# georgesterpu/avsr-tf1

Hardware: AMD Instinct MI355X
Metric: utterances/sec (train step) at B=64 T_a=500 T_v=75 (higher is better)
Workload: dtype f32; 1 GPU; c4: AV dual-attention (bimodal) video 1x256 + audio 3x256 uni-LSTM, scaled_luong, B=64 T_a=500x80 T_v=75 L=40; utterances_per_gpu=64, global_batch=64, T_a=500, F_a=80, T_v=75, F_v=128, T_dec=40, parallelism=dp1, video_frontend=resnet_cnn, launch=hipgraph, dropout=True

## Files before the change

avsr-tf1_amd/_lib.py:

```python
import ctypes as C
import os

import torch

from . import build as _build

MAX_LAYERS = 4
MAX_MECH = 4
MAX_STACKS = 4

_fp = C.POINTER(C.c_float)
_ip = C.POINTER(C.c_int32)


class AvsrError(RuntimeError):
    pass


class Mat(C.Structure):
    _fields_ = [("ptr", C.c_void_p), ("ld", C.c_int64), ("T", C.c_int32), ("pad_", C.c_int32), ("ldo", C.c_int64)]


class GemmDesc(C.Structure):
    _fields_ = [("A", Mat), ("B", Mat), ("C", Mat), ("bias", C.c_void_p),
# ... 4 lines not shown
                ("alpha_dev", C.c_void_p),
                ("splitk", C.c_int32), ("pad_", C.c_int32),
                ("workspace", C.c_void_p), ("workspace_floats", C.c_int64),
                ("colsum", C.c_void_p), ("colsum_beta", C.c_float), ("pad2_", C.c_int32)]


class RnnLayer(C.Structure):
    _fields_ = [("units", C.c_int32), ("in_dim", C.c_int32), ("hoisted", C.c_int32), ("out_col", C.c_int32),
                ("wt", C.c_void_p), ("w", C.c_void_p), ("bias", C.c_void_p),
                ("gates", C.c_void_p), ("cs", C.c_void_p), ("out", C.c_void_p), ("ld_out", C.c_int64),
                ("state", C.c_void_p), ("h_final", C.c_void_p), ("c_final", C.c_void_p),
                ("dgates", C.c_void_p), ("dstate", C.c_void_p), ("dout", C.c_void_p), ("ld_dout", C.c_int64),
                ("dout_col", C.c_int32), ("residual", C.c_int32), ("hs_seq", C.c_void_p), ("xt_seq", C.c_void_p),
                ("wt2", C.c_void_p), ("w2", C.c_void_p), ("bias2", C.c_void_p), ("rh_seq", C.c_void_p), ("dgates2", C.c_void_p)]


class RnnStack(C.Structure):
    _fields_ = [("B", C.c_int32), ("T", C.c_int32), ("reverse", C.c_int32), ("n_layers", C.c_int32),
                ("cell", C.c_int32), ("pad_", C.c_int32),
                ("len", C.c_void_p), ("dh_final", C.c_void_p), ("dc_final", C.c_void_p),
                ("seed", C.c_void_p), ("keep_in", C.c_float), ("keep_state", C.c_float), ("keep_out", C.c_float),
                ("consumer_keep", C.c_float), ("cell_id_base", C.c_int32), ("consumer_stream", C.c_int32),
                ("consumer_width", C.c_int32), ("pad2_", C.c_int32),
                ("layer", RnnLayer * MAX_LAYERS)]


class RnnLaunch(C.Structure):
    _fields_ = [(n, C.c_int32) for n in ("form", "stacks", "rows_per_group", "rows_per_slice", "launches", "wg_per_xcd", "crossing_edges",
                                         "top_tiles")]


class AttnMech(C.Structure):
    _fields_ = [("type", C.c_int32), ("T", C.c_int32), ("D", C.c_int32), ("chunk", C.c_int32),
                ("len", C.c_void_p), ("keys", C.c_void_p), ("values", C.c_void_p),
                ("values_sb", C.c_int64), ("values_st", C.c_int64),
                ("g", C.c_void_p), ("v", C.c_void_p), ("bq", C.c_void_p),
                ("wq_t", C.c_void_p), ("wq", C.c_void_p), ("watt_t", C.c_void_p), ("watt", C.c_void_p),
                ("scores", C.c_void_p), ("ctx", C.c_void_p), ("pq", C.c_void_p), ("pstat", C.c_void_p),
                ("pctx", C.c_void_p), ("dscores", C.c_void_p), ("dctx", C.c_void_p), ("dpq", C.c_void_p),
                ("pdq", C.c_void_p)]


class DecLayer(C.Structure):
    _fields_ = [("wt", C.c_void_p), ("w", C.c_void_p), ("bias", C.c_void_p), ("gates", C.c_void_p), ("cs", C.c_void_p),
                ("out", C.c_void_p), ("state", C.c_void_p), ("hs_seq", C.c_void_p), ("xin_seq", C.c_void_p),
                ("dgates", C.c_void_p), ("dstate", C.c_void_p), ("cell_id", C.c_int32), ("pad_", C.c_int32),
                ("wt2", C.c_void_p), ("w2", C.c_void_p), ("bias2", C.c_void_p), ("rh_seq", C.c_void_p), ("dgates2", C.c_void_p)]


MAX_DEC_EXTRA = 3


# ... 343 lines not shown
```

avsr-tf1_amd/csrc/persist.h:

```cpp
#pragma once
#include "common.h"
#include "wave.h"
#include "avsr_hip.h"

#define P_HDR 256

namespace avsr {

extern int32_t* g_sync;
extern int64_t g_sync_ints;
extern int g_persist_mode;
extern float* g_persist_scratch;
extern int64_t g_persist_scratch_floats;

struct RnnPlanRec { avsr_rnn_launch* out; int cap, n; };
extern thread_local RnnPlanRec* g_rnn_plan;
static inline void rnn_plan_note(int form, int stacks, int rows_per_group, int rows_per_slice, int B, int wg_per_xcd, int crossing = 0,
                                 int top_tiles = 0) {
  RnnPlanRec* R = g_rnn_plan;
  if (!R) return;
  if (R->n < R->cap)
    R->out[R->n] = avsr_rnn_launch{form, stacks, rows_per_group, rows_per_slice, (B + rows_per_slice - 1) / rows_per_slice, wg_per_xcd, crossing,
                                   top_tiles};
  ++R->n;
}

__device__ __forceinline__ f32x4 ld4_sc1(const float* p) {
  typedef unsigned long long u64;
  const u64 a = __hip_atomic_load(reinterpret_cast<const u64*>(p), __ATOMIC_RELAXED, __HIP_MEMORY_SCOPE_AGENT);
  const u64 b = __hip_atomic_load(reinterpret_cast<const u64*>(p) + 1, __ATOMIC_RELAXED, __HIP_MEMORY_SCOPE_AGENT);
  f32x4 v;
  v[0] = __builtin_bit_cast(float, (unsigned)(a & 0xffffffffu)); v[1] = __builtin_bit_cast(float, (unsigned)(a >> 32));
  v[2] = __builtin_bit_cast(float, (unsigned)(b & 0xffffffffu)); v[3] = __builtin_bit_cast(float, (unsigned)(b >> 32));
  return v;
}
__device__ __forceinline__ void st_sc1(float* p, float v) { __hip_atomic_store(p, v, __ATOMIC_RELAXED, __HIP_MEMORY_SCOPE_AGENT); }

__device__ __forceinline__ bool wait_ge(const int* ctr, int target, int* err) {
  for (int spins = 0; spins < (1 << 21); ++spins) {
    if (__hip_atomic_load(ctr, __ATOMIC_RELAXED, __HIP_MEMORY_SCOPE_AGENT) >= target) return true;
    if ((spins & 1023) == 1023 && __hip_atomic_load(err, __ATOMIC_RELAXED, __HIP_MEMORY_SCOPE_AGENT)) return false;
    __builtin_amdgcn_s_sleep(2);
  }
  __hip_atomic_store(err, 1, __ATOMIC_RELAXED, __HIP_MEMORY_SCOPE_AGENT);
  return false;
}
// ... 46 lines not shown
```

avsr-tf1_amd/csrc/rnn.hip:

```cpp
#include "step.h"
#include "avsr_hip.h"
#include "persist.h"

extern "C" int avsr_step_launch_raw(const void* launch, void* stream);
int avsr_rnn_fwd_persistent(const avsr_rnn_stack* st, int32_t n, void* stream, int dry);
int avsr_rnn_bwd_persistent(const avsr_rnn_stack* st, int32_t n, void* stream, int dry);

static int run_persistent(int (*fn)(const avsr_rnn_stack*, int32_t, void*, int), const avsr_rnn_stack* st, int32_t n, void* stream, int dry = 0) {
  for (int i = 0; i < n; ++i)
    for (int l = 0; l < st[i].n_layers && l < AVSR_MAX_LAYERS; ++l)
      if (st[i].layer[l].residual) return AVSR_ERR_UNSUPPORTED;
  int rc = fn(st, n, stream, dry);
  if (rc != AVSR_ERR_UNSUPPORTED || n == 1) return rc;
  avsr::RnnPlanRec* const rec = avsr::g_rnn_plan;
  const int noted = rec ? rec->n : 0;
  for (int i = 0; i < n; ++i)
    if ((rc = fn(st + i, 1, stream, 1)) != AVSR_OK) { if (rec) rec->n = noted; return rc; }
  if (dry) return AVSR_OK;
  for (int i = 0; i < n; ++i)
    if ((rc = fn(st + i, 1, stream, 0)) != AVSR_OK) return rc;
  return AVSR_OK;
}

static int wavefront_steps(const avsr_rnn_stack* st, int32_t n) {
// ... 290 lines not shown
  }
  return AVSR_OK;
}

extern "C" int avsr_rnn_plan(const avsr_rnn_stack* st, int32_t n, int32_t bwd, int32_t mode, int64_t sync_ints, int64_t scratch_floats,
                             avsr_rnn_launch* out, int32_t cap) {
  using namespace avsr;
  if (!st || n <= 0 || n > AVSR_MAX_STACKS || cap < 0 || (cap > 0 && !out) || sync_ints < 0 || scratch_floats < 0) return AVSR_ERR_ARG;
  for (int i = 0; i < n; ++i)
    if (st[i].n_layers <= 0 || st[i].n_layers > AVSR_MAX_LAYERS || st[i].B <= 0 || st[i].T <= 0) return AVSR_ERR_ARG;
  static int32_t dummy_sync[1];
  static float dummy_scratch[1];
  int32_t* const sync0 = g_sync; const int64_t ints0 = g_sync_ints; const int mode0 = g_persist_mode;
  float* const scr0 = g_persist_scratch; const int64_t floats0 = g_persist_scratch_floats;
  g_sync = sync_ints ? dummy_sync : nullptr; g_sync_ints = sync_ints; g_persist_mode = mode;
  g_persist_scratch = scratch_floats ? dummy_scratch : nullptr; g_persist_scratch_floats = scratch_floats;
  RnnPlanRec R = {out, cap, 0};
  g_rnn_plan = &R;
  const int rc = run_persistent(bwd ? avsr_rnn_bwd_persistent : avsr_rnn_fwd_persistent, st, n, nullptr, 1);
  g_rnn_plan = nullptr;
  g_sync = sync0; g_sync_ints = ints0; g_persist_mode = mode0; g_persist_scratch = scr0; g_persist_scratch_floats = floats0;
  if ((bwd || rc == AVSR_ERR_UNSUPPORTED) && wavefront_tasks(st, n) > STEP_MAX_TASKS) return AVSR_ERR_UNSUPPORTED;
  if (rc == AVSR_ERR_UNSUPPORTED) {
    if (cap > 0) out[0] = avsr_rnn_launch{AVSR_RNN_FORM_PER_STEP, n, 0, 0, wavefront_steps(st, n) * (st[0].cell == 1 ? 2 : 1), 0, 0, 0};
    return 1;
  }
  return rc < 0 ? rc : R.n;
}
```

avsr-tf1_amd/csrc/rnn_persist_bwd.hip:

```cpp
#include "step.h"
#include "avsr_hip.h"
#include "prof.h"
#include "persist.h"

#define B_MAX_TASKS 12
namespace avsr {
float* g_persist_scratch = nullptr;
int64_t g_persist_scratch_floats = 0;
}
extern "C" int avsr_rnn_set_persistent_scratch(float* scratch, int64_t floats) {
  avsr::g_persist_scratch = scratch; avsr::g_persist_scratch_floats = scratch ? floats : 0;
  return AVSR_OK;
}
#define B_CH 8

namespace avsr {

struct BTask {
  const float* w_own; const float* w_up; long ldw_own, ldw_up;
  const int* len;
  const float* gates; const float* cs;
  float* dgates; float* ring; const float* up_dgates;
  float* part;
  float* dx; int kind;
  const float* dout; long dout_sb, dout_st;
  const float* dh_final; const float* dc_final;
  int* prog; const int* prog_up;
  int* ctr; const int* ctr_up;
  int B, T, H, H_up, reverse, nct, nct_up, slot_begin, half, ntile, up_remote;
  const int32_t* seed; float k_st, k_out, k_in; uint32_t r_st, r_out, r_in; int in_W, in_coff;
};
struct BLaunch { int ntask, ngroups, wpx0, wpx1, b0, solo; int* err; int* claim; BTask task[B_MAX_TASKS]; };

__global__ __launch_bounds__(512) void rnn_persist_bwd_kernel(const BLaunch L) {
  __shared__ __attribute__((aligned(16))) float red[8][2][16][16];
  __shared__ int s_slot;
  const int tid = threadIdx.x, lane = tid & 63, wave = tid >> 6;
  const int xcc = __builtin_amdgcn_readfirstlane(xcc_id());
  if (tid == 0) s_slot = __hip_atomic_fetch_add(L.claim + xcc, 1, __ATOMIC_RELAXED, __HIP_MEMORY_SCOPE_AGENT);
  __syncthreads();
  const int slot = __builtin_amdgcn_readfirstlane(s_slot);
  const int g = xcc >> 1, half = xcc & 1;
  if (g >= L.ngroups || slot >= (half ? L.wpx1 : L.wpx0)) return;
  int ti = -1;
#pragma unroll
  for (int i = 0; i < B_MAX_TASKS; ++i)
    if (i < L.ntask && L.task[i].half == half && slot >= L.task[i].slot_begin) ti = i;
// ... 286 lines not shown
  auto publish = [&](int t) {
    asm volatile("s_waitcnt vmcnt(0)" ::: "memory");
    __syncthreads();
    if (tid == 0) {
      __hip_atomic_store(my_prog, T - t, __ATOMIC_RELAXED, __HIP_MEMORY_SCOPE_WORKGROUP);
      if (my_ctr) __hip_atomic_fetch_add(my_ctr + t, 1, __ATOMIC_RELAXED, __HIP_MEMORY_SCOPE_AGENT);
    }
  };

  if (helper) {
    const int K_up = 4 * tk.H_up, ncu = K_up >> 4;
    const int kw = wave & 7, tl = wave >> 3;
    const int b0 = (kw * ncu) / 8, nB = ((kw + 1) * ncu) / 8 - b0;
    f32x4 wB[B_CH];
    {
      const int uu = unit0 + tl * 16 + i;
#pragma unroll
      for (int c = 0; c < B_CH; ++c)
        wB[c] = (c < nB && uu < H) ? ld4(tk.w_up + (long)uu * tk.ldw_up + (b0 + c) * 16 + 4 * q) : f32x4{0.f, 0.f, 0.f, 0.f};
    }
    const __amdgpu_buffer_rsrc_t up_rs = make_rsrc(tk.up_dgates);
    const int up_row = (ab * T * K_up + b0 * 16 + 4 * q) * 4;
    float* const dx_p = tk.dx;
    const float k_in = tk.k_in; const uint32_t r_in = tk.r_in; const int in_W = tk.in_W, in_coff = tk.in_coff;
    for (int t = T - 1; t >= 0; --t) {
      wait_progress(0, t);
      lds_barrier();
      f32x4 aB[B_CH];
      const int o = (aok && t < len_a) ? up_row + (reverse ? len_a - 1 - t : t) * (K_up * 4) : P_OOB;
#pragma unroll
      for (int c = 0; c < B_CH; ++c) aB[c] = ldb_sc1(up_rs, c < nB ? o + c * 64 : P_OOB);
      f32x4 acc0 = {0.f, 0.f, 0.f, 0.f}, acc1 = {0.f, 0.f, 0.f, 0.f};
#pragma unroll
      for (int cc = 0; cc < B_CH; cc += 2)
#pragma unroll
        for (int e = 0; e < 4; ++e) {
          acc0 = __builtin_amdgcn_mfma_f32_16x16x4f32(aB[cc][e], wB[cc][e], acc0, 0, 0, 0);
          acc1 = __builtin_amdgcn_mfma_f32_16x16x4f32(aB[cc + 1][e], wB[cc + 1][e], acc1, 0, 0, 0);
        }
      acc0 += acc1;
#pragma unroll
      for (int r = 0; r < 4; ++r) red[wave][q * 4 + r][i] = acc0[r];
      lds_barrier();
      if (eok && t < len_b) {
        const int tau = reverse ? len_b - 1 - t : t;
        const long bt = (long)b * T + tau;
        float z = 0.f;
#pragma unroll
        for (int w = 0; w < 8; ++w) z += red[(eu >> 4) * 8 + w][er][eu & 15];
        const float v = z * p_drop(drop_on, seedv, r_in, (uint32_t)(bt * in_W + in_coff + u), k_in);
        if (publish_remote) st_sc1(dx_p + bt * H + u, v);
        else dx_p[bt * H + u] = v;
      }
      publish(t);
    }
    return;
  }

  f32x4 wR[TPW][KC];
#pragma unroll
  for (int nt = 0; nt < TPW; ++nt) {
    const int n = (wave * TPW + nt) * 16 + i;
#pragma unroll
    for (int c = 0; c < KC; ++c)
      wR[nt][c] = (n < H && unit0 * 4 + c * 16 + 4 * q < 4 * H) ? ld4(tk.w_own + (long)n * tk.ldw_own + unit0 * 4 + c * 16 + 4 * q)
                                                              : f32x4{0.f, 0.f, 0.f, 0.f};
  }
  float dc_carry = (eok && tk.dc_final) ? tk.dc_final[(long)b * H + u] : 0.f;
  float dh_carry = (eok && tk.dh_final) ? tk.dh_final[(long)b * H + u] : 0.f;
  const __amdgpu_buffer_rsrc_t gates_rs = make_rsrc(tk.gates), cs_rs = make_rsrc(tk.cs), dout_rs = make_rsrc(tk.dout);
  const __amdgpu_buffer_rsrc_t dx_rs = make_rsrc(tk.dx);
  const bool has_dout = tk.dout != nullptr, has_dx = tk.dx != nullptr;
  float* const dgates_p = tk.dgates;
  const __amdgpu_buffer_rsrc_t dgates_rs = make_rsrc(tk.dgates);
  const int dout_b = (int)(b * tk.dout_sb) + u, dout_st = (int)tk.dout_st;
  const float k_st = tk.k_st, k_out = tk.k_out;
  const uint32_t r_st = tk.r_st, r_out = tk.r_out;
// ... 132 lines not shown
  int best = -1, best_cross = 1 << 30, best_load = 1 << 30;
  for (int m = 0; m < (1 << n); ++m) {
    int load[2] = {0, 0}, cross = 0;
    for (int i = 0; i < n; ++i) {
      load[(m >> i) & 1] += cost[i];
      if (upper[i] >= 0 && (((m >> i) ^ (m >> upper[i])) & 1)) cross += ecost ? ecost[i] : 1;
    }
    if (load[0] > cap || load[1] > cap) continue;
    const int mx = load[0] > load[1] ? load[0] : load[1];
    if (cross < best_cross || (cross == best_cross && mx < best_load)) { best = m; best_cross = cross; best_load = mx; }
  }
  if (best < 0) return false;
  for (int i = 0; i < n; ++i) half_out[i] = (best >> i) & 1;
  return true;
}

static_assert(sizeof(BLaunch) <= 4000, "launch descriptor must fit the kernel-argument segment");

}

#include <cstdio>
#include <cstdlib>
#define UNSUP(code) do { if (getenv("AVSR_PERSIST_DEBUG")) fprintf(stderr, "[avsr] persistent BPTT not used: reason %d (rnn_persist_bwd.hip)\n", code); return AVSR_ERR_UNSUPPORTED; } while (0)
static int bwd_persistent(const avsr_rnn_stack* st, int32_t n, void* stream, int dry, bool ksplit);

int avsr_rnn_bwd_persistent(const avsr_rnn_stack* st, int32_t n, void* stream, int dry) {
  if (!(avsr::g_persist_mode & 4)) {
    const int rc = bwd_persistent(st, n, stream, dry, true);
    if (rc != AVSR_ERR_UNSUPPORTED) return rc;
  }
  return bwd_persistent(st, n, stream, dry, false);
}

static int bwd_persistent(const avsr_rnn_stack* st, int32_t n, void* stream, int dry, bool ksplit) {
  const int UWH = 16;
  using namespace avsr;
  int32_t* sync = g_sync; const int64_t sync_ints = g_sync_ints;
  if (!sync || !(g_persist_mode & 2)) return AVSR_ERR_UNSUPPORTED;
  if (ksplit && !g_persist_scratch) return AVSR_ERR_UNSUPPORTED;
  long part_used = 0;
  static thread_local BLaunch L;
  L = BLaunch{};
  double flops = 0.0;
  int cost[B_MAX_TASKS], upper[B_MAX_TASKS], half[B_MAX_TASKS];
  const int B = st[0].B;
  int ngroups = B < 64 ? (B + 15) / 16 : 4;
  for (int i = 0; i < n; ++i) {
    const avsr_rnn_stack& S = st[i];
    if (S.cell != 0 || S.B != B) UNSUP(3);
    const int first = L.ntask;
    for (int l = 0; l < S.n_layers; ++l) {
      const avsr_rnn_layer& Ly = S.layer[l];
      if (L.ntask >= B_MAX_TASKS) UNSUP(4);
      const int H = Ly.units, in = Ly.in_dim;
      const bool top = l + 1 >= S.n_layers;
      if (H % 16 || H > 32 * B_CH || (long)S.B * S.T * H * 4 >= (1L << 29)) UNSUP(5);
      if (!top && (S.layer[l + 1].units % 16 || S.layer[l + 1].units > 32 * B_CH || S.layer[l + 1].in_dim != H)) UNSUP(6);
      if (Ly.dout && (long)S.B * (S.T + 2) * Ly.ld_dout >= (1L << 29)) UNSUP(7);
      const int t_i = L.ntask++;
      BTask& tk = L.task[t_i];
      tk.w_own = Ly.w + (long)in * 4 * H; tk.ldw_own = 4 * H;
      if (!top && !ksplit) { const avsr_rnn_layer& Up = S.layer[l + 1]; tk.w_up = Up.w; tk.ldw_up = 4 * Up.units; tk.H_up = Up.units; tk.up_dgates = Up.dgates; }
      tk.len = S.len; tk.gates = Ly.gates; tk.cs = Ly.cs; tk.dgates = Ly.dgates; tk.ring = Ly.dstate;
      if (Ly.dout) { tk.dout = Ly.dout + Ly.ld_dout + Ly.dout_col; tk.dout_sb = (long)(S.T + 2) * Ly.ld_dout; tk.dout_st = Ly.ld_dout; }
      if (top) { tk.dh_final = S.dh_final; tk.dc_final = S.dc_final; }
      tk.B = S.B; tk.T = S.T; tk.H = H; tk.reverse = S.reverse;
      flops += 2.0 * S.B * S.T * (4.0 * H + (top ? 0.0 : 4.0 * S.layer[l + 1].units)) * H;
// ... 14 lines not shown
        if (!top && !ksplit) { tk.k_in = S.keep_in; tk.r_in = (cid + 1) * 4; tk.in_W = H; tk.in_coff = 0; }
      }
      if (ksplit && !top) {
        if (L.ntask >= B_MAX_TASKS) UNSUP(4);
        const avsr_rnn_layer& Up = S.layer[l + 1];
        const int h_i = L.ntask++;
        BTask& hk = L.task[h_i];
        hk.kind = 1;
        hk.w_up = Up.w; hk.ldw_up = 4 * Up.units; hk.H_up = Up.units; hk.up_dgates = Up.dgates;
        hk.len = S.len; hk.B = S.B; hk.T = S.T; hk.H = H; hk.reverse = S.reverse;
        hk.ntile = 1; hk.nct = H / UWH;
        const long need = (long)S.B * S.T * H;
        if (part_used + need > g_persist_scratch_floats) UNSUP(13);
        hk.dx = g_persist_scratch + part_used; part_used += need;
        tk.dx = hk.dx;
        cost[h_i] = hk.nct; upper[h_i] = h_i + 1;
        if (S.seed) {
          const uint32_t cid = (uint32_t)(S.cell_id_base + l);
          hk.seed = S.seed; hk.k_in = S.keep_in; hk.r_in = (cid + 1) * 4; hk.in_W = H; hk.in_coff = 0;
          hk.k_st = hk.k_out = 1.0f;
        }
      }
    }
    (void)first;
  }
  int ecost[B_MAX_TASKS];
  for (int i = 0; i < L.ntask; ++i) ecost[i] = L.task[i].kind == 1 ? 1 : 3;
  int total_cost = 0;
  for (int i = 0; i < L.ntask; ++i) total_cost += cost[i];
  const int cap = ksplit ? 64 : 28;
  const bool solo = ksplit && B > 64 && total_cost <= cap;
  if (solo) { for (int i = 0; i < L.ntask; ++i) half[i] = 0; ngroups = 8; }
  else if (!assign_halves(cost, upper, L.ntask, cap, half, ksplit ? ecost : nullptr)) UNSUP(9);
  long words = P_HDR + 8;
  int slots[2] = {0, 0};
  for (int pass = 0; pass < 2; ++pass)
    for (int i = 0; i < L.ntask; ++i) {
      BTask& tk = L.task[i];
      if ((tk.kind == 1) != (pass == 1)) continue;
      tk.half = half[i]; tk.slot_begin = slots[half[i]]; slots[half[i]] += tk.nct;
      tk.prog = sync + words; words += 8 * 32;
    }
  for (int i = 0; i < L.ntask; ++i) {
    BTask& tk = L.task[i];
    if (upper[i] < 0) continue;
    BTask& up = L.task[upper[i]];
    tk.prog_up = up.prog; tk.nct_up = up.nct;
    if (up.half != tk.half) {
      tk.up_remote = 1;
      if (!up.ctr) { up.ctr = sync + words; words += (long)ngroups * up.T; }
      tk.ctr_up = up.ctr;
    }
  }
  if (words > sync_ints) UNSUP(10);
  const int slice = solo ? 128 : 64;
  const int wpx = slots[0] > slots[1] ? slots[0] : slots[1];
  if (dry) {
    int crossing = 0, tiles = 1;
    for (int i = 0; i < L.ntask; ++i) { crossing += L.task[i].up_remote; if (L.task[i].ntile > tiles) tiles = L.task[i].ntile; }
    rnn_plan_note(!ksplit ? AVSR_RNN_FORM_BWD_UNIT : solo ? AVSR_RNN_FORM_BWD_KSPLIT_SOLO : AVSR_RNN_FORM_BWD_KSPLIT, n, 16, slice, B, wpx, crossing,
                  ksplit ? 0 : tiles);
    return AVSR_OK;
  }
  L.err = sync; L.claim = sync + P_HDR; L.wpx0 = slots[0]; L.wpx1 = slots[1]; L.solo = solo ? 1 : 0;
  hipStream_t s = (hipStream_t)stream;
  for (int b0 = 0; b0 < B; b0 += slice) {
    const int rows = B - b0 < slice ? B - b0 : slice;
    L.b0 = b0; L.ngroups = (rows + 15) / 16;
    if (avsr::dev_zero(sync + P_HDR, sizeof(int32_t) * (words - P_HDR), s) != hipSuccess) return AVSR_ERR_HIP;
    {
      ProfScope ps(PROF_RNN_PERSIST_BWD, s, flops * rows / B);
      if (ksplit) hipLaunchKernelGGL(rnn_persist_bwdk_kernel, dim3(8 * wpx), dim3(512), 0, s, L);
      else hipLaunchKernelGGL(rnn_persist_bwd_kernel, dim3(8 * wpx), dim3(512), 0, s, L);
    }
    AVSR_CHECK_LAUNCH();
  }
  return AVSR_OK;
}
```

avsr-tf1_amd/model_encoder.py:

```python
import torch
from . import ops
from ._lib import RnnStack
from .config import encoder_cell_id
from .model_base import Batch


class EncoderMixin:
    def _kn(self, prefix):
        return (prefix + "/gates_kernel", prefix + "/gates_bias") if self.gru else (prefix + "/kernel", prefix + "/bias")

    def _keeps(self, s):
        return self.cfg.video_dropout if s == "video" else self.cfg.audio_dropout

    def _sdrop(self, s):
        return self._dropping and min(self._keeps(s)) < 1.0

    def _bdrop(self, blk):
        return self._dropping and min(blk["keep"]) < 1.0

    def _rnn_stack(self, ws, s, d, B, len_t, backward=False):
        cfg = self.cfg
        E = ws["enc"][s]
        st = RnnStack()
        st.B, st.T, st.reverse, st.n_layers, st.cell = B, E["T"], int(d == "bw"), E["nplain"], int(self.gru)
# ... 19 lines not shown
            Ly.w = ops.fptr(self.params, self.P[name].off)
            Ly.bias = ops.fptr(self.params, self.P[bname].off)
            if self.gru:
                cn = f"{s}/enc/{d}/l{cfg.shared_layer(s, l)}/cand_kernel"
                Ly.wt2, Ly.w2 = ops.fptr(self.derived, self.Tr[cn].off), ops.fptr(self.params, self.P[cn].off)
                Ly.bias2 = ops.fptr(self.params, self.P[f"{s}/enc/{d}/l{cfg.shared_layer(s, l)}/cand_bias"].off)
                Ly.rh_seq, Ly.dgates2 = ops.fptr(Ld["rh"]), ops.fptr(Ld["dpc"])
            Ly.gates, Ly.cs = ops.fptr(Ld["gates"]), ops.fptr(Ld["cs"])
            Ly.out, Ly.ld_out = ops.fptr(Ld["out"].t), Ld["out"].D
            Ly.state, Ly.h_final, Ly.c_final = ops.fptr(Ld["state"]), ops.fptr(Ld["hf"]), ops.fptr(Ld["cf"])
            Ly.dgates, Ly.dstate = ops.fptr(Ld["dgates"]), ops.fptr(Ld["dstate"])
            Ly.residual = int(cfg.residual(s) and l > 0)
            if drop or Ly.residual:
                Ly.hs_seq = ops.fptr(Ld["hs_seq"].t)
            if drop:
                if "xt_seq" in Ld:
                    Ly.xt_seq = ops.fptr(Ld["xt_seq"].t)
            if backward and Ld["dout"] is not None:
                Ly.dout, Ly.ld_dout, Ly.dout_col = ops.fptr(Ld["dout"].t), Ld["dout"].D, Ld["col"]
            i = u
        if backward and not E["attentive"]:
            top = E["layers"][(d, E["nplain"] - 1)]
            st.dh_final, st.dc_final = ops.fptr(top["dhf"]), (None if self.gru else ops.fptr(top["dcf"]))
        return st

    def _rnn_stack_single(self, ws, s, d, l, B, len_t, backward=False):
        cfg = self.cfg
        E = ws["enc"][s]
        Ld = E["layers"][(d, l)]
        u = E["units"][l]
        st = RnnStack()
        st.B, st.T, st.reverse, st.n_layers, st.cell = B, E["T"], int(d == "bw"), 1, int(self.gru)
        st.len = ops.fptr(len_t)
        drop = self._sdrop(s)
        if drop:
            st.seed = ops.fptr(self.seed)
            st.keep_in, st.keep_state, st.keep_out = self._keeps(s)
            st.cell_id_base = encoder_cell_id(s, d, l)
        name, bname = self._kn(f"{s}/enc/{d}/l{l}")
        Ly = st.layer[0]
        Ly.units, Ly.in_dim, Ly.hoisted = u, (E["F0"] if l == 0 else u), 1
        Ly.wt, Ly.w = ops.fptr(self.derived, self.Tr[name].off), ops.fptr(self.params, self.P[name].off)
        Ly.bias = ops.fptr(self.params, self.P[bname].off)
        if self.gru:
            cn = f"{s}/enc/{d}/l{l}/cand_kernel"
            Ly.wt2, Ly.w2 = ops.fptr(self.derived, self.Tr[cn].off), ops.fptr(self.params, self.P[cn].off)
            Ly.bias2 = ops.fptr(self.params, self.P[f"{s}/enc/{d}/l{l}/cand_bias"].off)
# ... 318 lines not shown
            self._encode_highway(ws, B)
        for s in cfg.streams():
            E = ws["enc"][s]
            if E["attentive"]:
                self._av_align_forward(ws, batch, training)
                continue
            self._final_state_fwd(ws, s)
            if s == "video" and cfg.regress_aus and training:
                Wau = self.P["video/au/kernel"]
                ops.gemm(E["mem"].mat(), Wau.mat(2), ops.mat(E["au_z"], 2), B * E["T"], 2, E["mem"].D, bias=self._pp("video/au/bias"))
                ops.au_loss(E["au_z"], batch.aus, E["len"], E["au_row"], E["au_dz"], B, E["T"], cfg.au_loss_weight * self.au_scale,
                            total_count=self.au_total if self.au_external else None)

    @staticmethod
    def _run_stacks(stacks, fn):
        if not stacks:
            return
        if sum(s.n_layers for s in stacks) <= 8 and len(stacks) <= 4:
            fn(stacks)
            return
        for s in stacks:
            fn([s])

    def _pp(self, name):
        r = self.P[name]
        return r.t[r.off:r.off + r.n]

    def _gp(self, name):
        r = self.Gr[name]
        return r.t[r.off:r.off + r.n]

    def _final_state_fwd(self, ws, s):
        cfg, B = self.cfg, ws["B"]
        E = ws["enc"][s]
        top = len(E["units"]) - 1
        u, H = E["units"][-1], cfg.decoder_units[0]
        if cfg.encoder_type == "unidirectional":
            Lt = E["layers"][("fw", top)]
            E["c_fin"], E["h_fin"] = (None if self.gru else Lt["cf"]), Lt["hf"]
            return
        for nm, key, dst in ((("proj", "hf", "h_dec"),) if self.gru else (("proj_c", "cf", "c_dec"), ("proj_h", "hf", "h_dec"))):
            Pm = self.P[f"{s}/enc/{nm}"]
            for di, d in enumerate(cfg.directions()):
                ops.gemm(ops.mat(E["layers"][(d, top)][key], u), Pm.mat(H, row0=di * u), ops.mat(E[dst], H), B, H, u,
                         beta=0.0 if di == 0 else 1.0)
        E["c_fin"], E["h_fin"] = (None if self.gru else E["c_dec"]), E["h_dec"]
# ... 26 lines not shown
        if "video" in ws["enc"] and cfg.regress_aus:
            E = ws["enc"]["video"]
            T, D = E["T"], E["mem"].D
            ops.gemm(ops.mat(E["au_dz"], 2), self.P["video/au/kernel"].mat(2), E["dmem"].mat(), B * T, D, 2, trans_b=1, beta=1.0)
            self._gemm_tn(E["mem"].mat(), ops.mat(E["au_dz"], 2), self.Gr["video/au/kernel"].mat(2), D, 2, B * T)
            ops.colsum(ops.mat(E["au_dz"], 2), B * T, 2, self.grads, self.scratch, beta=1.0, out_offset=self.Gr["video/au/bias"].off)
        if cfg.use_ctc:
            s = cfg.ctc_stream()
            E, md = ws["enc"][s], self._mem_desc(ws, s)
            T, D, Cc = E["T"], cfg.memory_depth(s), cfg.vocab_size + 1
            dzm = ops.mat(E["ctc_dz"], Cc)
            ops.gemm(dzm, self.P[f"{s}/ctc/kernel"].mat(Cc), md["gmat"], B * T, D, Cc, trans_b=1, beta=1.0)
            self._gemm_tn(md["vmat"], dzm, self.Gr[f"{s}/ctc/kernel"].mat(Cc), D, Cc, B * T)
            ops.colsum(dzm, B * T, Cc, self.grads, self.scratch, beta=1.0, out_offset=self.Gr[f"{s}/ctc/bias"].off)
        if cfg.architecture == "av_align":
            self._av_align_backward(ws, batch)
        stacks = []
        for s in cfg.streams():
            E = ws["enc"][s]
            if E["nplain"] == 0 or cfg.highway(s):
                continue
            for d in cfg.directions():
                stacks.append(self._rnn_stack(ws, s, d, B, E["len"], backward=True))
        self._run_stacks(stacks, ops.rnn_bwd)
        if any(cfg.highway(s) for s in cfg.streams()):
            self._encode_highway_backward(ws, B)
        for s in cfg.streams():
            E = ws["enc"][s]
            T, F, F0 = E["T"], E["F"], E["F0"]
            first = True
            for d in cfg.directions():
                i = F0
                for l in range(0 if cfg.highway(s) else E["nplain"]):
                    u = E["units"][l]
                    Ld = E["layers"][(d, l)]
                    kname, bname = self._kn(f"{s}/enc/{d}/l{cfg.shared_layer(s, l)}")
                    Gk = self.Gr[kname]
                    G = self.G
                    dg = ops.mat(Ld["dgates"], G * u)
                    drop = self._sdrop(s)
                    if l == 0:
                        a_x = ops.mat(E["xd"][d] if drop else E["xin0"], F0)
                    elif drop:
                        a_x = E["layers"][(d, l - 1)]["xt_seq"].mat(0)
                    else:
                        a_x = E["layers"][(d, l - 1)]["out"].mat(0, E["layers"][(d, l - 1)]["col"])
                    nct = (G * u + 127) // 128
                    gt = (((i + 127) // 128) + ((u + 127) // 128)) * nct if not self.gru else None
                    with ops.gemm_group():
                        self._gemm_tn(a_x, dg, Gk.mat(G * u), i, G * u, B * T, group_tiles=gt)
                        sh = 1 if d == "bw" else -1
                        a_h = Ld["hs_seq"].mat(sh) if (drop or (cfg.residual(s) and l > 0)) else Ld["out"].mat(sh, Ld["col"])
                        self._gemm_tn(a_h, dg, Gk.mat(G * u, row0=i), u, G * u, B * T, colsum=(self.grads, self.Gr[bname].off), group_tiles=gt)
                        if self.gru:
                            Gc = self.Gr[f"{s}/enc/{d}/l{cfg.shared_layer(s, l)}/cand_kernel"]
                            dpc = ops.mat(Ld["dpc"], u)
                            self._gemm_tn(a_x, dpc, Gc.mat(u), i, u, B * T)
                            self._gemm_tn(ops.mat(Ld["rh"], u), dpc, Gc.mat(u, row0=i), u, u, B * T)
                            ops.colsum(dpc, B * T, u, self.grads, self.scratch, beta=1.0, out_offset=self.Gr[f"{s}/enc/{d}/l{cfg.shared_layer(s, l)}/cand_bias"].off)
                    i = u
                if E["nplain"] > 0 and (cfg.batch_normalisation or "cnn" in E or self.n_dense or cfg.instance_normalisation):
                    u0, G = E["units"][0], self.G
                    W0 = self.P[self._kn(f"{s}/enc/{d}/l0")[0]]
                    L0 = E["layers"][(d, 0)]
                    tgt = E["dx_tmp"] if self._sdrop(s) else E["dxin0"]
                    beta0 = 0.0 if (self._sdrop(s) or first) else 1.0
                    ops.gemm(ops.mat(L0["dgates"], G * u0), W0.mat(G * u0), ops.mat(tgt, F0), B * T, F0, G * u0, trans_b=1, beta=beta0)
                    if self.gru:
                        ops.gemm(ops.mat(L0["dpc"], u0), self.P[f"{s}/enc/{d}/l0/cand_kernel"].mat(u0), ops.mat(tgt, F0), B * T, F0, u0,
                                 trans_b=1, beta=1.0)
                    if self._sdrop(s):
                        ops.dropout_rows(ops.mat(E["dx_tmp"], F0), ops.mat(E["dxin0"], F0), B * T, F0, self.seed,
                                         encoder_cell_id(s, d, 0) * 4, self._keeps(s)[0], F0, accumulate=not first)
                    first = False
            if self.n_dense:
                for k in reversed(range(self.n_dense)):
                    Dn, u = E["dense"][k], cfg.input_dense_layers[k]
                    a_prev, w_prev = (E["dense"][k - 1]["a"], cfg.input_dense_layers[k - 1]) if k else (E["xin"], F)
                    ops.selu_bwd(Dn["z"], Dn["da"], Dn["z"], B * T * u)
                    self._gemm_tn(ops.mat(a_prev, w_prev), ops.mat(Dn["z"], u), self.Gr[f"{s}/dense{k}/kernel"].mat(u), w_prev, u, B * T)
                    g_prev = E["dense"][k - 1]["da"] if k else E["dxn"]
                    ops.gemm(ops.mat(Dn["z"], u), self.P[f"{s}/dense{k}/kernel"].mat(u), ops.mat(g_prev, w_prev), B * T, w_prev, u, trans_b=1)
            if cfg.instance_normalisation:
                ops.instnorm_bwd(E["in_x"], E["dxn"], self._pp(f"{s}/in/gamma"), E["in_mean"], E["in_invstd"], E["dxn"], E["in_dg"], E["in_db"],
# ... 29 lines not shown
```

avsr-tf1_amd/ops.py:

```python
import ctypes as C
import os

import torch

from . import _lib
from ._lib import (AttnMech, AttnRnn, GemmDesc, Mat, RnnLayer, RnnStack, TransposeJob, check, stream_ptr)


def fptr(t, offset=0):
    if t is None:
        return None
    assert t.is_cuda, "HIP engine buffers must live on the GPU"
    return t.data_ptr() + t.element_size() * int(offset)


def mat(t, ld, T=0, ldo=0, offset=0):
    assert t.dtype == torch.float32
    return Mat(fptr(t, offset), int(ld), int(T), 0, int(ldo))


def _L():
    return _lib.load()


# ... 112 lines not shown
    arr = (RnnStack * len(stacks))(*stacks)
    check(_L().avsr_rnn_bwd(arr, len(stacks), _s()), "avsr_rnn_bwd")


RNN_FORMS = ("per_step", "fwd_xcd8", "fwd_xcd8_q4", "fwd_xcd16", "fwd_parts", "fwd_agent", "bwd_ksplit", "bwd_ksplit_solo", "bwd_unit")


def rnn_plan(stacks, bwd=False, mode=3, sync_ints=1 << 20, scratch_floats=64 << 20):
    from ._lib import RnnLaunch
    arr = (RnnStack * len(stacks))(*stacks)
    out = (RnnLaunch * MAX_STACKS_PLAN)()
    n = _L().avsr_rnn_plan(arr, len(stacks), int(bool(bwd)), int(mode), int(sync_ints), int(scratch_floats), out, MAX_STACKS_PLAN)
    if n < 0:
        check(n, "avsr_rnn_plan")
    recs = [{f: getattr(out[i], f) for f, _ in RnnLaunch._fields_} for i in range(n)]
    for r in recs:
        r["form"] = RNN_FORMS[r["form"]]
    return recs


MAX_STACKS_PLAN = 4


def attn_rnn_fwd(desc, l_begin, l_end):
    check(_L().avsr_attn_rnn_fwd(C.byref(desc), int(l_begin), int(l_end), _s()), "avsr_attn_rnn_fwd")


def attn_rnn_bwd(desc):
    check(_L().avsr_attn_rnn_bwd(C.byref(desc), _s()), "avsr_attn_rnn_bwd")


def beam_search_step(logits, n_utt, beam_width, V, step, eos_id, length_penalty_weight, logp_in, fin_in, len_in, logp_out, fin_out, len_out,
                     tok, parent_rows, step_ids, parent_ids, n_unfinished, x=None, x_stride=0, O=0, wout_t=None, bout=None):
    check(_L().avsr_beam_search_step(fptr(logits), n_utt, beam_width, V, step, eos_id, float(length_penalty_weight), fptr(logp_in), fptr(fin_in),
                                     fptr(len_in), fptr(logp_out), fptr(fin_out), fptr(len_out), fptr(tok), fptr(parent_rows), fptr(step_ids),
                                     fptr(parent_ids), fptr(n_unfinished), fptr(x), x_stride, O, fptr(wout_t), fptr(bout), _s()),
          "avsr_beam_search_step")


def beam_search_step_lm(logits, n_utt, beam_width, V, step, eos_id, length_penalty_weight, logp_in, fin_in, len_in, logp_out, fin_out, len_out,
                        tok, parent_rows, step_ids, parent_ids, n_unfinished, lm_logp, lm_weight, x=None, x_stride=0, O=0, wout_t=None, bout=None):
    check(_L().avsr_beam_search_step_lm(fptr(logits), n_utt, beam_width, V, step, eos_id, float(length_penalty_weight), fptr(logp_in), fptr(fin_in),
                                        fptr(len_in), fptr(logp_out), fptr(fin_out), fptr(len_out), fptr(tok), fptr(parent_rows), fptr(step_ids),
                                        fptr(parent_ids), fptr(n_unfinished), fptr(x), x_stride, O, fptr(wout_t), fptr(bout), fptr(lm_logp),
                                        float(lm_weight), _s()), "avsr_beam_search_step_lm")

# ... 361 lines not shown
    check(_L().avsr_optimiser_step(fptr(params), fptr(grads), fptr(m), fptr(v), n, fptr(gnorm), fptr(step), float(lr),
                                   int(warmup_steps), int(first_decay_steps), float(clip_norm), float(grad_scale), OPTIMISER[optimiser],
                                   float(weight_decay), _s()), "avsr_optimiser_step")


PROF_KINDS = ("gemm", "step_lstm_fwd", "step_lstm_bwd", "step_dense", "attn_fwd", "attn_bwd", "rnn_persist_fwd", "rnn_persist_bwd", "dec_persist_fwd", "dec_persist_bwd",
              "conv_fwd", "conv_bwd_data", "conv_bwd_weight", "align_persist_fwd", "align_persist_bwd")


def prof_begin(max_launches=65536):
    check(_L().avsr_prof_begin(int(max_launches)), "avsr_prof_begin")


def prof_end():
    cnt = (C.c_int32 * len(PROF_KINDS))()
    ms = (C.c_float * len(PROF_KINDS))()
    fl = (C.c_double * len(PROF_KINDS))()
    check(_L().avsr_prof_end(cnt, ms, fl), "avsr_prof_end")
    return {k: (int(cnt[i]), float(ms[i]), float(fl[i])) for i, k in enumerate(PROF_KINDS)}


_persist_sync = None
_persist_scratch = None


def rnn_set_persistent(on, device="cuda", ints=1 << 20, mode=3, scratch_floats=64 << 20):
    global _persist_sync, _persist_scratch
    check(_L().avsr_rnn_set_persistent_mode(int(mode)), "avsr_rnn_set_persistent_mode")
    if on:
        if _persist_sync is None:
            _persist_sync = torch.zeros(ints, dtype=torch.int32, device=device)
        if (mode & 6) == 2 and _persist_scratch is None:
            _persist_scratch = torch.zeros(scratch_floats, dtype=torch.float32, device=device)
        if _persist_scratch is not None:
            check(_L().avsr_rnn_set_persistent_scratch(_persist_scratch.data_ptr(), _persist_scratch.numel()), "avsr_rnn_set_persistent_scratch")
        _persist_sync[:1].zero_()
        check(_L().avsr_rnn_set_persistent(_persist_sync.data_ptr(), ints), "avsr_rnn_set_persistent")
    else:
        check(_L().avsr_rnn_set_persistent(None, 0), "avsr_rnn_set_persistent")


def rnn_persistent_clear():
    if _persist_sync is not None:
        _persist_sync[:1].zero_()


def attn_rnn_fused_ws_floats(B, n_mech, Dmax=256):
    return int(_L().avsr_attn_rnn_fused_ws_floats(int(B), int(n_mech), int(Dmax)))


# ... 290 lines not shown
```

include/avsr_hip.h:

```cpp
#ifndef AVSR_HIP_H
#define AVSR_HIP_H
#include <stdint.h>

#ifdef __cplusplus
extern "C" {
#endif
#if defined(__GNUC__) || defined(__clang__)
#pragma GCC visibility push(default)
#endif

#define AVSR_OK 0
#define AVSR_ERR_ARG (-1)
#define AVSR_ERR_HIP (-2)
#define AVSR_ERR_UNSUPPORTED (-3)

#define AVSR_MAX_LAYERS 4
#define AVSR_MAX_MECH 4
#define AVSR_MAX_STACKS 4
#define AVSR_HAVE_ATTN 1
#define AVSR_MAX_TRANSPOSE 16
#define AVSR_MAX_SEGMENTS 32

int avsr_abi_version(void);
int64_t avsr_sizeof(const char* name);
// ... 43 lines not shown
  float* dstate;
  const float* dout;
  int64_t ld_dout;
  int32_t dout_col;
  int32_t residual;
  float* hs_seq;
  float* xt_seq;
  const float* wt2;
  const float* w2;
  const float* bias2;
  float* rh_seq;
  float* dgates2;
} avsr_rnn_layer;

typedef struct avsr_rnn_stack {
  int32_t B, T, reverse, n_layers;
  int32_t cell, pad_;
  const int32_t* len;
  const float* dh_final;
  const float* dc_final;
  const int32_t* seed;
  float keep_in, keep_state, keep_out, consumer_keep;
  int32_t cell_id_base, consumer_stream, consumer_width, pad2_;
  avsr_rnn_layer layer[AVSR_MAX_LAYERS];
} avsr_rnn_stack;

int avsr_rnn_fwd(const avsr_rnn_stack* stacks, int32_t n_stacks, void* stream);
int avsr_rnn_bwd(const avsr_rnn_stack* stacks, int32_t n_stacks, void* stream);

int avsr_rnn_set_persistent(int32_t* sync, int64_t ints);
int avsr_rnn_set_persistent_mode(int mode);
int avsr_rnn_set_persistent_scratch(float* scratch, int64_t floats);
#define AVSR_RNN_FORM_PER_STEP 0
#define AVSR_RNN_FORM_FWD_XCD8 1
#define AVSR_RNN_FORM_FWD_XCD8_Q4 2
#define AVSR_RNN_FORM_FWD_XCD16 3
#define AVSR_RNN_FORM_FWD_PARTS 4
#define AVSR_RNN_FORM_FWD_AGENT 5
#define AVSR_RNN_FORM_BWD_KSPLIT 6
#define AVSR_RNN_FORM_BWD_KSPLIT_SOLO 7
#define AVSR_RNN_FORM_BWD_UNIT 8
typedef struct avsr_rnn_launch {
  int32_t form, stacks, rows_per_group, rows_per_slice;
  int32_t launches, wg_per_xcd, crossing_edges, top_tiles;
} avsr_rnn_launch;
int avsr_rnn_plan(const avsr_rnn_stack* stacks, int32_t n_stacks, int32_t bwd, int32_t mode, int64_t sync_ints, int64_t scratch_floats,
                  avsr_rnn_launch* out, int32_t cap);

typedef struct avsr_attn_mech {
  int32_t type;
  int32_t T, D, chunk;
  const int32_t* len;
  const float* keys;
  const float* values;
  int64_t values_sb, values_st;
  const float* g;
  const float* v;
  const float* bq;
  const float* wq_t;
  const float* wq;
  const float* watt_t;
  const float* watt;
  float* scores;
  float* ctx;
  float* pq;
  float* pstat;
  float* pctx;
// ... 535 lines not shown
```

Baseline: 5713 utterances/sec.

## Fold encoder layer-0 input-gradient GEMM into persistent BPTT kernel as trailing task

Adds an optional trailing task to the persistent backward RNN kernel that computes the layer-0 input gradient (dxin0) step by step as dgates become available, including dropout masking and zeroing past sequence length. The separate post-BPTT GEMM for dxin0 is then skipped for streams where the plan reports the trailing task ran. This overlaps the input-gradient work with the sequential recurrence instead of running it afterwards, at the cost of extra work slots and wavefronts in the persistent kernel plus a host-side plan query per backward call.

```diff
diff --git a/avsr-tf1_amd/_lib.py b/avsr-tf1_amd/_lib.py
--- a/avsr-tf1_amd/_lib.py
+++ b/avsr-tf1_amd/_lib.py
@@ -50,12 +50,13 @@
                 ("seed", C.c_void_p), ("keep_in", C.c_float), ("keep_state", C.c_float), ("keep_out", C.c_float),
                 ("consumer_keep", C.c_float), ("cell_id_base", C.c_int32), ("consumer_stream", C.c_int32),
                 ("consumer_width", C.c_int32), ("pad2_", C.c_int32),
+                ("dxin0", C.c_void_p),
                 ("layer", RnnLayer * MAX_LAYERS)]
 
 
 class RnnLaunch(C.Structure):
     _fields_ = [(n, C.c_int32) for n in ("form", "stacks", "rows_per_group", "rows_per_slice", "launches", "wg_per_xcd", "crossing_edges",
-                                         "top_tiles")]
+                                         "top_tiles", "trailing")]
 
 
 class AttnMech(C.Structure):
diff --git a/avsr-tf1_amd/csrc/persist.h b/avsr-tf1_amd/csrc/persist.h
--- a/avsr-tf1_amd/csrc/persist.h
+++ b/avsr-tf1_amd/csrc/persist.h
@@ -16,12 +16,12 @@
 struct RnnPlanRec { avsr_rnn_launch* out; int cap, n; };
 extern thread_local RnnPlanRec* g_rnn_plan;
 static inline void rnn_plan_note(int form, int stacks, int rows_per_group, int rows_per_slice, int B, int wg_per_xcd, int crossing = 0,
-                                 int top_tiles = 0) {
+                                 int top_tiles = 0, int trailing = 0) {
   RnnPlanRec* R = g_rnn_plan;
   if (!R) return;
   if (R->n < R->cap)
     R->out[R->n] = avsr_rnn_launch{form, stacks, rows_per_group, rows_per_slice, (B + rows_per_slice - 1) / rows_per_slice, wg_per_xcd, crossing,
-                                   top_tiles};
+                                   top_tiles, trailing};
   ++R->n;
 }
 
diff --git a/avsr-tf1_amd/csrc/rnn.hip b/avsr-tf1_amd/csrc/rnn.hip
--- a/avsr-tf1_amd/csrc/rnn.hip
+++ b/avsr-tf1_amd/csrc/rnn.hip
@@ -336,7 +336,7 @@
   g_sync = sync0; g_sync_ints = ints0; g_persist_mode = mode0; g_persist_scratch = scr0; g_persist_scratch_floats = floats0;
   if ((bwd || rc == AVSR_ERR_UNSUPPORTED) && wavefront_tasks(st, n) > STEP_MAX_TASKS) return AVSR_ERR_UNSUPPORTED;
   if (rc == AVSR_ERR_UNSUPPORTED) {
-    if (cap > 0) out[0] = avsr_rnn_launch{AVSR_RNN_FORM_PER_STEP, n, 0, 0, wavefront_steps(st, n) * (st[0].cell == 1 ? 2 : 1), 0, 0, 0};
+    if (cap > 0) out[0] = avsr_rnn_launch{AVSR_RNN_FORM_PER_STEP, n, 0, 0, wavefront_steps(st, n) * (st[0].cell == 1 ? 2 : 1), 0, 0, 0, 0};
     return 1;
   }
   return rc < 0 ? rc : R.n;
diff --git a/avsr-tf1_amd/csrc/rnn_persist_bwd.hip b/avsr-tf1_amd/csrc/rnn_persist_bwd.hip
--- a/avsr-tf1_amd/csrc/rnn_persist_bwd.hip
+++ b/avsr-tf1_amd/csrc/rnn_persist_bwd.hip
@@ -23,6 +23,7 @@
   float* dgates; float* ring; const float* up_dgates;
   float* part;
   float* dx; int kind;
+  int trail;
   const float* dout; long dout_sb, dout_st;
   const float* dh_final; const float* dc_final;
   int* prog; const int* prog_up;
@@ -355,6 +356,7 @@
     const __amdgpu_buffer_rsrc_t up_rs = make_rsrc(tk.up_dgates);
     const int up_row = (ab * T * K_up + b0 * 16 + 4 * q) * 4;
     float* const dx_p = tk.dx;
+    const bool trail = tk.trail != 0;
     const float k_in = tk.k_in; const uint32_t r_in = tk.r_in; const int in_W = tk.in_W, in_coff = tk.in_coff;
     for (int t = T - 1; t >= 0; --t) {
       wait_progress(0, t);
@@ -384,8 +386,10 @@
         const float v = z * p_drop(drop_on, seedv, r_in, (uint32_t)(bt * in_W + in_coff + u), k_in);
         if (publish_remote) st_sc1(dx_p + bt * H + u, v);
         else dx_p[bt * H + u] = v;
-      }
-      publish(t);
+      } else if (trail && eok) {
+        dx_p[((long)b * T + t) * H + u] = 0.f;
+      }
+      if (!trail) publish(t);
     }
     return;
   }
@@ -564,17 +568,23 @@
 #include <cstdio>
 #include <cstdlib>
 #define UNSUP(code) do { if (getenv("AVSR_PERSIST_DEBUG")) fprintf(stderr, "[avsr] persistent BPTT not used: reason %d (rnn_persist_bwd.hip)\n", code); return AVSR_ERR_UNSUPPORTED; } while (0)
-static int bwd_persistent(const avsr_rnn_stack* st, int32_t n, void* stream, int dry, bool ksplit);
+static int bwd_persistent(const avsr_rnn_stack* st, int32_t n, void* stream, int dry, bool ksplit, bool trailing);
 
 int avsr_rnn_bwd_persistent(const avsr_rnn_stack* st, int32_t n, void* stream, int dry) {
   if (!(avsr::g_persist_mode & 4)) {
-    const int rc = bwd_persistent(st, n, stream, dry, true);
+    bool want = false;
+    for (int i = 0; i < n; ++i) want = want || st[i].dxin0 != nullptr;
+    if (want && !(avsr::g_persist_mode & 8)) {
+      const int rc = bwd_persistent(st, n, stream, dry, true, true);
+      if (rc != AVSR_ERR_UNSUPPORTED) return rc;
+    }
+    const int rc = bwd_persistent(st, n, stream, dry, true, false);
     if (rc != AVSR_ERR_UNSUPPORTED) return rc;
   }
-  return bwd_persistent(st, n, stream, dry, false);
-}
-
-static int bwd_persistent(const avsr_rnn_stack* st, int32_t n, void* stream, int dry, bool ksplit) {
+  return bwd_persistent(st, n, stream, dry, false, false);
+}
+
+static int bwd_persistent(const avsr_rnn_stack* st, int32_t n, void* stream, int dry, bool ksplit, bool trailing) {
   const int UWH = 16;
   using namespace avsr;
   int32_t* sync = g_sync; const int64_t sync_ints = g_sync_ints;
@@ -585,6 +595,7 @@
   L = BLaunch{};
   double flops = 0.0;
   int cost[B_MAX_TASKS], upper[B_MAX_TASKS], half[B_MAX_TASKS];
+  int cell0[AVSR_MAX_STACKS], trail_mask = 0;
   const int B = st[0].B;
   int ngroups = B < 64 ? (B + 15) / 16 : 4;
   for (int i = 0; i < n; ++i) {
@@ -645,8 +656,32 @@
         }
       }
     }
-    (void)first;
-  }
+    cell0[i] = first;
+  }
+  for (int i = 0; trailing && i < n; ++i) {
+    const avsr_rnn_stack& S = st[i];
+    const avsr_rnn_layer& L0 = S.layer[0];
+    const int in = L0.in_dim;
+    if (!S.dxin0 || in <= 0 || in % 16 || in > 256 || L.ntask >= B_MAX_TASKS) continue;
+    bool shared = false;
+    for (int j = 0; j < n; ++j) shared = shared || (j != i && st[j].dxin0 == S.dxin0);
+    if (shared) continue;
+    const int h_i = L.ntask++;
+    BTask& hk = L.task[h_i];
+    hk.kind = 1; hk.trail = 1;
+    hk.w_up = L0.w; hk.ldw_up = 4 * L0.units; hk.H_up = L0.units; hk.up_dgates = L0.dgates;
+    hk.len = S.len; hk.B = S.B; hk.T = S.T; hk.H = in; hk.reverse = S.reverse;
+    hk.ntile = 1; hk.nct = in / UWH;
+    hk.dx = S.dxin0;
+    cost[h_i] = hk.nct; upper[h_i] = cell0[i];
+    if (S.seed) {
+      hk.seed = S.seed; hk.k_in = S.keep_in; hk.r_in = (uint32_t)S.cell_id_base * 4; hk.in_W = in; hk.in_coff = 0;
+      hk.k_st = hk.k_out = 1.0f;
+    }
+    flops += 2.0 * S.B * S.T * 4.0 * L0.units * in;
+    trail_mask |= 1 << i;
+  }
+  if (trailing && !trail_mask) return AVSR_ERR_UNSUPPORTED;
   int ecost[B_MAX_TASKS];
   for (int i = 0; i < L.ntask; ++i) ecost[i] = L.task[i].kind == 1 ? 1 : 3;
   int total_cost = 0;
@@ -657,10 +692,10 @@
   else if (!assign_halves(cost, upper, L.ntask, cap, half, ksplit ? ecost : nullptr)) UNSUP(9);
   long words = P_HDR + 8;
   int slots[2] = {0, 0};
-  for (int pass = 0; pass < 2; ++pass)
+  for (int pass = 0; pass < 3; ++pass)
     for (int i = 0; i < L.ntask; ++i) {
       BTask& tk = L.task[i];
-      if ((tk.kind == 1) != (pass == 1)) continue;
+      if ((tk.kind == 1 ? 1 + tk.trail : 0) != pass) continue;
       tk.half = half[i]; tk.slot_begin = slots[half[i]]; slots[half[i]] += tk.nct;
       tk.prog = sync + words; words += 8 * 32;
     }
@@ -682,7 +717,7 @@
     int crossing = 0, tiles = 1;
     for (int i = 0; i < L.ntask; ++i) { crossing += L.task[i].up_remote; if (L.task[i].ntile > tiles) tiles = L.task[i].ntile; }
     rnn_plan_note(!ksplit ? AVSR_RNN_FORM_BWD_UNIT : solo ? AVSR_RNN_FORM_BWD_KSPLIT_SOLO : AVSR_RNN_FORM_BWD_KSPLIT, n, 16, slice, B, wpx, crossing,
-                  ksplit ? 0 : tiles);
+                  ksplit ? 0 : tiles, trail_mask);
     return AVSR_OK;
   }
   L.err = sync; L.claim = sync + P_HDR; L.wpx0 = slots[0]; L.wpx1 = slots[1]; L.solo = solo ? 1 : 0;
diff --git a/avsr-tf1_amd/model_encoder.py b/avsr-tf1_amd/model_encoder.py
--- a/avsr-tf1_amd/model_encoder.py
+++ b/avsr-tf1_amd/model_encoder.py
@@ -65,7 +65,13 @@
         if backward and not E["attentive"]:
             top = E["layers"][(d, E["nplain"] - 1)]
             st.dh_final, st.dc_final = ops.fptr(top["dhf"]), (None if self.gru else ops.fptr(top["dcf"]))
+        if backward and self._needs_dxin0(E) and len(cfg.directions()) == 1 and not self.gru:
+            st.dxin0 = ops.fptr(E["dxin0"])
         return st
+
+    def _needs_dxin0(self, E):
+        cfg = self.cfg
+        return E["nplain"] > 0 and bool(cfg.batch_normalisation or "cnn" in E or self.n_dense or cfg.instance_normalisation)
 
     def _rnn_stack_single(self, ws, s, d, l, B, len_t, backward=False):
         cfg = self.cfg
@@ -430,6 +436,17 @@
         for s in stacks:
             fn([s])
 
+    @staticmethod
+    def _run_stacks_bwd(stacks):
+        if not stacks:
+            return set()
+        calls = [stacks] if (sum(s.n_layers for s in stacks) <= 8 and len(stacks) <= 4) else [[s] for s in stacks]
+        done = set()
+        for call in calls:
+            done |= {st._stream for st, t in zip(call, ops.rnn_bwd_trailing(call)) if t}
+            ops.rnn_bwd(call)
+        return done
+
     def _pp(self, name):
         r = self.P[name]
         return r.t[r.off:r.off + r.n]
@@ -502,7 +519,8 @@
                 continue
             for d in cfg.directions():
                 stacks.append(self._rnn_stack(ws, s, d, B, E["len"], backward=True))
-        self._run_stacks(stacks, ops.rnn_bwd)
+                stacks[-1]._stream = s
+        dx_done = self._run_stacks_bwd(stacks)
         if any(cfg.highway(s) for s in cfg.streams()):
             self._encode_highway_backward(ws, B)
         for s in cfg.streams():
@@ -539,7 +557,7 @@
                             self._gemm_tn(ops.mat(Ld["rh"], u), dpc, Gc.mat(u, row0=i), u, u, B * T)
                             ops.colsum(dpc, B * T, u, self.grads, self.scratch, beta=1.0, out_offset=self.Gr[f"{s}/enc/{d}/l{cfg.shared_layer(s, l)}/cand_bias"].off)
                     i = u
-                if E["nplain"] > 0 and (cfg.batch_normalisation or "cnn" in E or self.n_dense or cfg.instance_normalisation):
+                if self._needs_dxin0(E) and s not in dx_done:
                     u0, G = E["units"][0], self.G
                     W0 = self.P[self._kn(f"{s}/enc/{d}/l0")[0]]
                     L0 = E["layers"][(d, 0)]
diff --git a/avsr-tf1_amd/ops.py b/avsr-tf1_amd/ops.py
--- a/avsr-tf1_amd/ops.py
+++ b/avsr-tf1_amd/ops.py
@@ -158,6 +158,17 @@
 MAX_STACKS_PLAN = 4
 
 
+def rnn_bwd_trailing(stacks):
+    on, mode, ints = _persist_state
+    if not on or not any(st.dxin0 for st in stacks):
+        return [False] * len(stacks)
+    floats = _persist_scratch.numel() if _persist_scratch is not None else 0
+    recs = rnn_plan(stacks, bwd=True, mode=mode, sync_ints=ints, scratch_floats=floats)
+    if len(recs) == 1:
+        return [bool(recs[0]["trailing"] >> i & 1) for i in range(len(stacks))]
+    return [bool(r["trailing"] & 1) for r in recs]
+
+
 def attn_rnn_fwd(desc, l_begin, l_end):
     check(_L().avsr_attn_rnn_fwd(C.byref(desc), int(l_begin), int(l_end), _s()), "avsr_attn_rnn_fwd")
 
@@ -565,10 +576,12 @@
 
 _persist_sync = None
 _persist_scratch = None
+_persist_state = (False, 3, 0)
 
 
 def rnn_set_persistent(on, device="cuda", ints=1 << 20, mode=3, scratch_floats=64 << 20):
-    global _persist_sync, _persist_scratch
+    global _persist_sync, _persist_scratch, _persist_state
+    _persist_state = (bool(on), int(mode), int(ints) if on else 0)
     check(_L().avsr_rnn_set_persistent_mode(int(mode)), "avsr_rnn_set_persistent_mode")
     if on:
         if _persist_sync is None:
diff --git a/include/avsr_hip.h b/include/avsr_hip.h
--- a/include/avsr_hip.h
+++ b/include/avsr_hip.h
@@ -89,6 +89,7 @@
   const int32_t* seed;
   float keep_in, keep_state, keep_out, consumer_keep;
   int32_t cell_id_base, consumer_stream, consumer_width, pad2_;
+  float* dxin0;
   avsr_rnn_layer layer[AVSR_MAX_LAYERS];
 } avsr_rnn_stack;
 
@@ -110,6 +111,7 @@
 typedef struct avsr_rnn_launch {
   int32_t form, stacks, rows_per_group, rows_per_slice;
   int32_t launches, wg_per_xcd, crossing_edges, top_tiles;
+  int32_t trailing;
 } avsr_rnn_launch;
 int avsr_rnn_plan(const avsr_rnn_stack* stacks, int32_t n_stacks, int32_t bwd, int32_t mode, int64_t sync_ints, int64_t scratch_floats,
                   avsr_rnn_launch* out, int32_t cap);
```

New measurement: 5740 utterances/sec (median of 4 runs). Within noise of the previous version (+0.5%).
